# weiyithu/PV-RAFT

Hardware: NVIDIA H100
Metric: raft_sample_iters_per_sec (higher is better)
Workload: dtype f32

## Files before the change

### pvraft_b200/csrc/corr_gemm.cu

```cuda
#include "tma.cuh"
#include "wgmma.cuh"

namespace pvraft {

constexpr int kGemmThreads = 384;
constexpr int kTileM = 128, kTileN = 128, kBlockK = 32;
constexpr int kOperandBytes = kTileM * kBlockK * 4;
constexpr int kStageBytes = 4 * kOperandBytes;
constexpr int kStages = 3;
constexpr int kConsumerWarps = 8;

struct GemmParams {
    float* corr;
    int N, M, C;
    float scale;
    float rscale;
    int r0, c0;
    int tiles_m, tiles_n;
    long long ldc;
    long long n_tiles;
};

__device__ __forceinline__ float div_by_const(float x, float s, float r) {
    const float q0 = x * r;
    return fmaf(fmaf(-q0, s, x), r, q0);
}

__global__ void __launch_bounds__(kGemmThreads, 1)
k_corr_gemm(const __grid_constant__ CUtensorMap map_a_hi, const __grid_constant__ CUtensorMap map_a_lo,
            const __grid_constant__ CUtensorMap map_b_hi, const __grid_constant__ CUtensorMap map_b_lo, const GemmParams p) {
    extern __shared__ __align__(1024) unsigned char smem_raw[];
    unsigned char* tiles = SMEM_ALIGN_1024(smem_raw);
    __shared__ __align__(8) unsigned long long s_full[kStages], s_empty[kStages];
    const int warp = warp_id(), lane = lane_id();
    const int num_kb = p.C / kBlockK;
    const long long my_tiles = blockIdx.x < p.n_tiles ? (p.n_tiles - 1 - blockIdx.x) / gridDim.x + 1 : 0;

    if (warp == 0 && lane == 0) {
        prefetch_tensormap(&map_a_hi);
        prefetch_tensormap(&map_a_lo);
        prefetch_tensormap(&map_b_hi);
        prefetch_tensormap(&map_b_lo);
        for (int s = 0; s < kStages; ++s) { mbar_init(&s_full[s], 1); mbar_init(&s_empty[s], kConsumerWarps); }
        fence_mbarrier_init();
    }
    __syncthreads();
    const int tiles_per_batch = p.tiles_m * p.tiles_n;

    if (warp < 4) {
        if (warp == 0 && lane == 0) {
            int s = 0;
            unsigned phase = 0;
            for (long long i = 0; i < my_tiles; ++i) {
                const long long t = blockIdx.x + i * gridDim.x;
                const int b = (int)(t / tiles_per_batch), r = (int)(t - (long long)b * tiles_per_batch);
                const int tile_m = r / p.tiles_n, tile_n = r - tile_m * p.tiles_n;
                const int row_a = b * p.N + p.r0 + tile_m * kTileM, row_b = b * p.M + p.c0 + tile_n * kTileN;
                for (int kb = 0; kb < num_kb; ++kb) {
                    mbar_wait(&s_empty[s], phase ^ 1u);
                    unsigned char* st = tiles + (size_t)s * kStageBytes;
                    mbar_expect_tx(&s_full[s], kStageBytes);
                    tma_load_2d(st + 0 * kOperandBytes, &map_a_hi, &s_full[s], kb * kBlockK, row_a);
                    tma_load_2d(st + 1 * kOperandBytes, &map_a_lo, &s_full[s], kb * kBlockK, row_a);
                    tma_load_2d(st + 2 * kOperandBytes, &map_b_hi, &s_full[s], kb * kBlockK, row_b);
                    tma_load_2d(st + 3 * kOperandBytes, &map_b_lo, &s_full[s], kb * kBlockK, row_b);
                    if (++s == kStages) { s = 0; phase ^= 1u; }
                }
            }
        }
        return;
    }
    const int half = (warp >> 2) - 1;
    const int wq = warp & 3;
    const int a_off = half * 64 * 128;
    float acc[64];
    int s = 0, prev_s = -1;
    unsigned phase = 0;
    for (long long i = 0; i < my_tiles; ++i) {
        const long long t = blockIdx.x + i * gridDim.x;
        const int b = (int)(t / tiles_per_batch), r = (int)(t - (long long)b * tiles_per_batch);
        const int tile_m = r / p.tiles_n, tile_n = r - tile_m * p.tiles_n;
        for (int kb = 0; kb < num_kb; ++kb) {
            mbar_wait(&s_full[s], phase);
            unsigned char* st = tiles + (size_t)s * kStageBytes;
            const unsigned long long a_hi = wgmma_desc(st + 0 * kOperandBytes + a_off), a_lo = wgmma_desc(st + 1 * kOperandBytes + a_off);
            const unsigned long long b_hi = wgmma_desc(st + 2 * kOperandBytes), b_lo = wgmma_desc(st + 3 * kOperandBytes);
            wgmma_fence_regs(acc);
            wgmma_fence();
#pragma unroll
            for (int k = 0; k < kBlockK / 8; ++k) {
                wgmma_tf32<kTileN>(acc, wgmma_desc_k(a_hi, k), wgmma_desc_k(b_hi, k), (kb | k) != 0);
                wgmma_tf32<kTileN>(acc, wgmma_desc_k(a_lo, k), wgmma_desc_k(b_hi, k), 1);
                wgmma_tf32<kTileN>(acc, wgmma_desc_k(a_hi, k), wgmma_desc_k(b_lo, k), 1);
            }
            wgmma_commit();
            wgmma_wait<1>();
            if (prev_s >= 0 && lane == 0) mbar_arrive(&s_empty[prev_s]);
            prev_s = s;
            if (++s == kStages) { s = 0; phase ^= 1u; }
        }
        wgmma_wait<0>();
        wgmma_fence_regs(acc);
        if (lane == 0) mbar_arrive(&s_empty[prev_s]);
        prev_s = -1;
        const int row = tile_m * kTileM + half * 64 + wq * 16 + (lane >> 2);
        float* o = p.corr + ((size_t)b * p.tiles_m * kTileM + row) * (size_t)p.ldc + (size_t)tile_n * kTileN + 2 * (lane & 3);
        const size_t down8 = (size_t)8 * p.ldc;
#pragma unroll
        for (int j = 0; j < kTileN / 8; ++j) {
            *reinterpret_cast<float2*>(o + 8 * j) = make_float2(div_by_const(acc[4 * j + 0], p.scale, p.rscale), div_by_const(acc[4 * j + 1], p.scale, p.rscale));
            *reinterpret_cast<float2*>(o + down8 + 8 * j) = make_float2(div_by_const(acc[4 * j + 2], p.scale, p.rscale), div_by_const(acc[4 * j + 3], p.scale, p.rscale));
        }
    }
}

__global__ void k_tf32_split(const float* __restrict__ x, long long n, float* __restrict__ hi, float* __restrict__ lo) {
    const long long i = ((long long)blockIdx.x * blockDim.x + threadIdx.x) * 4;
    if (i >= n) return;
    const float4 v = *reinterpret_cast<const float4*>(x + i);
    float h[4], l[4];
    const float in[4] = {v.x, v.y, v.z, v.w};
#pragma unroll
    for (int q = 0; q < 4; ++q) {
        unsigned hb, lb;
        asm("cvt.rna.tf32.f32 %0, %1;" : "=r"(hb) : "f"(in[q]));
        h[q] = __uint_as_float(hb);
        asm("cvt.rna.tf32.f32 %0, %1;" : "=r"(lb) : "f"(in[q] - h[q]));
        l[q] = __uint_as_float(lb);
    }
    *reinterpret_cast<float4*>(hi + i) = make_float4(h[0], h[1], h[2], h[3]);
    *reinterpret_cast<float4*>(lo + i) = make_float4(l[0], l[1], l[2], l[3]);
}

static int launch_gemm(const float* a_hi, const float* a_lo, const float* b_hi, const float* b_lo, int B, int N, int M, int C, int r0,
                       int tiles_m, int c0, int tiles_n, float* corr, long long ldc, cudaStream_t st) {
    int rc;
    CUtensorMap ma_hi, ma_lo, mb_hi, mb_lo;
    const long long rows_a = (long long)B * N, rows_b = (long long)B * M;
    if ((rc = make_tensor_map(&ma_hi, a_hi, rows_a, C, C, kTileM, "corr_matmul")) ||
        (rc = make_tensor_map(&ma_lo, a_lo, rows_a, C, C, kTileM, "corr_matmul")) ||
        (rc = make_tensor_map(&mb_hi, b_hi, rows_b, C, C, kTileN, "corr_matmul")) ||
        (rc = make_tensor_map(&mb_lo, b_lo, rows_b, C, C, kTileN, "corr_matmul")))
        return rc;
    GemmParams p{};
    p.corr = corr; p.N = N; p.M = M; p.C = C;
    p.scale = sqrtf((float)C);
    p.rscale = (float)(1.0 / (double)p.scale);
    p.r0 = r0; p.c0 = c0;
    p.tiles_m = tiles_m; p.tiles_n = tiles_n;
    p.ldc = ldc;
    p.n_tiles = (long long)B * tiles_m * tiles_n;
    const size_t smem = (size_t)kStages * kStageBytes + 1024;
    if ((rc = opt_in_smem(k_corr_gemm, smem))) return rc;
    const int grid = (int)(p.n_tiles < sm_count() ? p.n_tiles : sm_count());
    k_corr_gemm<<<grid, kGemmThreads, smem, st>>>(ma_hi, ma_lo, mb_hi, mb_lo, p);
    return check_launch("corr_gemm");
}

static void launch_split(const float* x, long long n, float* hi, float* lo, cudaStream_t st) {
    k_tf32_split<<<(unsigned)((n / 4 + 255) / 256), 256, 0, st>>>(x, n, hi, lo);
}

}

using namespace pvraft;

extern "C" int64_t pvraft_corr_matmul_workspace_bytes(int B, int N, int M, int C) {
    if (B <= 0 || N <= 0 || M <= 0 || C <= 0) return 0;
    return (int64_t)2 * B * ((int64_t)N + M) * C * (int64_t)sizeof(float);
}

extern "C" int pvraft_corr_matmul_fwd(const float* fmap1, const float* fmap2, int B, int N, int M, int C, float* corr, void* workspace,
                                      void* stream) {
    if (!fmap1 || !fmap2 || !corr || !workspace) return fail(PVRAFT_ERR_BAD_ARG, "corr_matmul: null pointer");
    if (B <= 0 || N <= 0 || M <= 0 || C <= 0) return fail(PVRAFT_ERR_BAD_ARG, "corr_matmul: bad shape");
    if (N % kTileM || M % kTileN || C % kBlockK)
        return fail(PVRAFT_ERR_UNSUPPORTED, "corr_matmul: N=%d and M=%d must be multiples of 128 and C=%d of 32", N, M, C);
    if (B > 65535 || N / kTileM > 65535 || M / kTileN > 65535) return fail(PVRAFT_ERR_UNSUPPORTED, "corr_matmul: grid too large");
    cudaStream_t st = (cudaStream_t)stream;
    const long long na = (long long)B * N * C, nb = (long long)B * M * C;
    float* a_hi = reinterpret_cast<float*>(workspace);
    float* a_lo = a_hi + na;
    float* b_hi = a_lo + na;
    float* b_lo = b_hi + nb;
    launch_split(fmap1, na, a_hi, a_lo, st);
    launch_split(fmap2, nb, b_hi, b_lo, st);
    const int rc = check_launch("tf32_split");
    if (rc) return rc;
    return launch_gemm(a_hi, a_lo, b_hi, b_lo, B, N, M, C, 0, N / kTileM, 0, M / kTileN, corr, M, st);
}

extern "C" int pvraft_tf32_split_fwd(const float* x, int64_t n, float* hi, float* lo, void* stream) {
    if (!x || !hi || !lo || n <= 0) return fail(PVRAFT_ERR_BAD_ARG, "tf32_split: bad argument");
    if (n % 4 || ((uintptr_t)x | (uintptr_t)hi | (uintptr_t)lo) % 16)
        return fail(PVRAFT_ERR_UNSUPPORTED, "tf32_split: n=%lld must be a multiple of 4 and the buffers 16-byte aligned", (long long)n);
    launch_split(x, n, hi, lo, (cudaStream_t)stream);
    return check_launch("tf32_split");
}

extern "C" int pvraft_corr_matmul_window_fwd(const float* a_hi, const float* a_lo, const float* b_hi, const float* b_lo, int B, int N,
                                             int M, int C, int r0, int rows, int c0, int cols, float* corr, int64_t ldc, void* stream) {
    if (!a_hi || !a_lo || !b_hi || !b_lo || !corr) return fail(PVRAFT_ERR_BAD_ARG, "corr_matmul_window: null pointer");
    if (B <= 0 || N <= 0 || M <= 0 || C <= 0 || rows <= 0 || cols <= 0 || r0 < 0 || c0 < 0)
        return fail(PVRAFT_ERR_BAD_ARG, "corr_matmul_window: bad shape");
    if (N % kTileM || M % kTileN || C % kBlockK || r0 % kTileM || c0 % kTileN)
        return fail(PVRAFT_ERR_UNSUPPORTED, "corr_matmul_window: N=%d, M=%d, r0=%d and c0=%d must be multiples of 128 and C=%d of 32", N,
                    M, r0, c0, C);
    const int tiles_m = (rows + kTileM - 1) / kTileM, tiles_n = (cols + kTileN - 1) / kTileN;
    if (rows > N - r0 || cols > M - c0 || r0 + tiles_m * kTileM > N || c0 + tiles_n * kTileN > M)
        return fail(PVRAFT_ERR_UNSUPPORTED, "corr_matmul_window: rows [%d, %d) x columns [%d, %d), whole tiles, exceed N=%d x M=%d", r0,
                    r0 + tiles_m * kTileM, c0, c0 + tiles_n * kTileN, N, M);
    if (ldc < (int64_t)tiles_n * kTileN || ldc % 4)
        return fail(PVRAFT_ERR_UNSUPPORTED, "corr_matmul_window: ldc=%lld (need a multiple of 4, >= %d)", (long long)ldc, tiles_n * kTileN);
    if ((long long)B * N > 0x7fffffffLL || (long long)B * M > 0x7fffffffLL)
        return fail(PVRAFT_ERR_UNSUPPORTED, "corr_matmul_window: B*N=%lld / B*M=%lld operand rows", (long long)B * N, (long long)B * M);
    return launch_gemm(a_hi, a_lo, b_hi, b_lo, B, N, M, C, r0, tiles_m, c0, tiles_n, corr, ldc, (cudaStream_t)stream);
}
```

### pvraft_b200/csrc/corr_topk.cu

```cuda
#include "common.cuh"

namespace pvraft {

constexpr int kTopkThreads = 256;

__device__ __forceinline__ int padded(int i) { return i + (i >> 5); }

__global__ void __launch_bounds__(kTopkThreads) k_corr_topk(const float* __restrict__ corr, int M, long long ld, int K,
                                                            float* __restrict__ val, int32_t* __restrict__ idx, long long ld_out,
                                                            int col_base, const int32_t* __restrict__ ids) {
    extern __shared__ __align__(16) unsigned char smem_raw[];
    unsigned* s_key = reinterpret_cast<unsigned*>(smem_raw);
    __shared__ int s_hist[256];
    __shared__ unsigned s_prefix, s_need;
    __shared__ unsigned s_warp[kTopkThreads / 32];
    const size_t row = blockIdx.x;
    const float* src = corr + row * (size_t)ld;
    const int tid = threadIdx.x, lane = tid & 31, w = tid >> 5;
    for (int i = tid; i < M; i += kTopkThreads) s_key[padded(i)] = ord_key(__ldg(src + i));
    if (tid == 0) { s_prefix = 0u; s_need = (unsigned)K; }
    for (int pass = 0; pass < 4; ++pass) {
        const int shift = 24 - 8 * pass;
        s_hist[tid] = 0;
        __syncthreads();
        const unsigned prefix = s_prefix;
        const unsigned mask = pass == 0 ? 0u : (0xFFFFFFFFu << (shift + 8));
        for (int i = tid; i < M; i += kTopkThreads) {
            const unsigned k = s_key[padded(i)];
            if ((k & mask) == prefix) atomicAdd(&s_hist[(k >> shift) & 0xFF], 1);
        }
        __syncthreads();
        if (w == 0) {
            int h[8], mine = 0;
#pragma unroll
            for (int q = 0; q < 8; ++q) { h[q] = s_hist[lane * 8 + q]; mine += h[q]; }
            int above = mine;
#pragma unroll
            for (int o = 1; o < 32; o <<= 1) {
                const int a = __shfl_down_sync(kFull, above, o);
                if (lane + o < 32) above += a;
            }
            const int need = (int)s_need;
            const int higher = above - mine;
            const bool here = higher < need && above >= need;
            if (here) {
                int acc = higher, bin = 7;
                for (; bin > 0; --bin) {
                    if (acc + h[bin] >= need) break;
                    acc += h[bin];
                }
                s_need = (unsigned)(need - acc);
                s_prefix = prefix | ((unsigned)(lane * 8 + bin) << shift);
            }
        }
        __syncthreads();
    }
    const unsigned T = s_prefix;
    const int need_eq = (int)s_need;
    const int seg = (M + kTopkThreads - 1) / kTopkThreads;
    const int c0 = tid * seg, c1 = min(M, c0 + seg);
    unsigned n_gt = 0, n_eq = 0;
    for (int i = c0; i < c1; ++i) {
        const unsigned k = s_key[padded(i)];
        n_gt += k > T ? 1u : 0u;
        n_eq += k == T ? 1u : 0u;
    }
    unsigned packed = n_gt | (n_eq << 16), incl = packed;
#pragma unroll
    for (int o = 1; o < 32; o <<= 1) {
        const unsigned a = __shfl_up_sync(kFull, incl, o);
        if (lane >= o) incl += a;
    }
    if (lane == 31) s_warp[w] = incl;
    __syncthreads();
    unsigned base = 0;
    for (int q = 0; q < w; ++q) base += s_warp[q];
    const unsigned excl = base + incl - packed;
    const int gt_before = (int)(excl & 0xFFFFu), eq_before = (int)(excl >> 16);
    int pos = gt_before + min(eq_before, need_eq);
    int eq_seen = eq_before;
    for (int i = c0; i < c1; ++i) {
        const unsigned k = s_key[padded(i)];
        bool keep = k > T;
        if (k == T) { keep = eq_seen < need_eq; ++eq_seen; }
        if (keep) {
            val[row * ld_out + pos] = ord_float(k);
            idx[row * ld_out + pos] = ids ? __ldg(ids + row * ld + i) : col_base + i;
            ++pos;
        }
    }
}

__global__ void __launch_bounds__(kTopkThreads) k_corr_topk_vec(const float* __restrict__ corr, int M, long long ld, int K,
                                                                float* __restrict__ val, int32_t* __restrict__ idx, long long ld_out,
                                                                int col_base, const int32_t* __restrict__ ids) {
    extern __shared__ __align__(16) unsigned char smem_raw[];
    uint4* s_key = reinterpret_cast<uint4*>(smem_raw);
    constexpr int kCand = 1024;
    __shared__ int s_hist[2048 + kTopkThreads];
    __shared__ unsigned s_cand[kCand];
    __shared__ int s_wsum[kTopkThreads / 32];
    __shared__ unsigned s_scan[kTopkThreads / 32][7];
    __shared__ unsigned s_prefix;
    __shared__ int s_need;
    const int tid = threadIdx.x, lane = tid & 31, w = tid >> 5;
    const size_t row = blockIdx.x;
    const float4* src = reinterpret_cast<const float4*>(corr + row * (size_t)ld);
#pragma unroll
    for (int j = 0; j < 8; ++j) {
        const int c4 = j * kTopkThreads + tid;
        uint4 kk = make_uint4(0u, 0u, 0u, 0u);
        if (c4 * 4 < M) {
            const float4 v = __ldg(src + c4);
            kk = make_uint4(ord_key(v.x), ord_key(v.y), ord_key(v.z), ord_key(v.w));
        }
        s_key[c4] = kk;
    }
    const int sink = 2048 + tid;
    auto find_bin = [&](unsigned prefix, int shift, int need) {
        int h[8], mine = 0;
#pragma unroll
        for (int q = 0; q < 8; ++q) { h[q] = s_hist[tid * 8 + q]; mine += h[q]; }
        int incl = mine;
#pragma unroll
        for (int o = 1; o < 32; o <<= 1) {
            const int a = __shfl_down_sync(kFull, incl, o);
            if (lane + o < 32) incl += a;
        }
        if (lane == 0) s_wsum[w] = incl;
        __syncthreads();
        int above = incl;
        for (int ww = w + 1; ww < kTopkThreads / 32; ++ww) above += s_wsum[ww];
        const int higher = above - mine;
        if (higher < need && above >= need) {
            int acc = higher, bin = 7;
            for (; bin > 0; --bin) {
                if (acc + h[bin] >= need) break;
                acc += h[bin];
            }
            s_need = need - acc;
            s_prefix = prefix | ((unsigned)(tid * 8 + bin) << shift);
        }
        __syncthreads();
    };
    for (int i = tid; i < 2048; i += kTopkThreads) s_hist[i] = 0;
    __syncthreads();
#pragma unroll
    for (int j = 0; j < 8; ++j) {
        const uint4 kk = s_key[j * kTopkThreads + tid];
        atomicAdd(&s_hist[kk.x >> 21], 1);
        atomicAdd(&s_hist[kk.y >> 21], 1);
        atomicAdd(&s_hist[kk.z >> 21], 1);
        atomicAdd(&s_hist[kk.w >> 21], 1);
    }
    __syncthreads();
    find_bin(0u, 21, K);
    unsigned prefix = s_prefix;
    int need = s_need;
    int ncand = 0;
    {
        const unsigned top = prefix >> 21;
        int mine = 0;
#pragma unroll
        for (int j = 0; j < 8; ++j) {
            const uint4 kk = s_key[j * kTopkThreads + tid];
            mine += ((kk.x >> 21) == top) + ((kk.y >> 21) == top) + ((kk.z >> 21) == top) + ((kk.w >> 21) == top);
        }
        int incl = mine;
#pragma unroll
        for (int o = 1; o < 32; o <<= 1) {
            const int a = __shfl_up_sync(kFull, incl, o);
            if (lane >= o) incl += a;
        }
        if (lane == 31) s_wsum[w] = incl;
        __syncthreads();
        int at = incl - mine, total = 0;
        for (int ww = 0; ww < kTopkThreads / 32; ++ww) {
            const int a = s_wsum[ww];
            total += a;
            if (ww < w) at += a;
        }
        ncand = total;
        if (total <= kCand && mine > 0) {
#pragma unroll
            for (int j = 0; j < 8; ++j) {
                const uint4 kk = s_key[j * kTopkThreads + tid];
                const unsigned ke[4] = {kk.x, kk.y, kk.z, kk.w};
#pragma unroll
                for (int e = 0; e < 4; ++e) {
                    const bool hit = (ke[e] >> 21) == top;
                    if (hit) s_cand[at] = ke[e];
                    at += hit ? 1 : 0;
                }
            }
        }
    }
    __syncthreads();
#pragma unroll 1
    for (int pass = 1; pass < 3; ++pass) {
        const int shift = pass == 1 ? 10 : 0;
        const unsigned digit_mask = pass == 1 ? 0x7FFu : 0x3FFu;
        const unsigned hi_mask = 0xFFFFFFFFu << (shift + (pass == 1 ? 11 : 10));
        for (int i = tid; i < 2048; i += kTopkThreads) s_hist[i] = 0;
        __syncthreads();
        if (ncand <= kCand) {
            for (int i = tid; i < ncand; i += kTopkThreads) {
                const unsigned k = s_cand[i];
                atomicAdd(&s_hist[(k & hi_mask) == prefix ? (int)((k >> shift) & digit_mask) : sink], 1);
            }
        } else {
#pragma unroll
            for (int j = 0; j < 8; ++j) {
                const uint4 kk = s_key[j * kTopkThreads + tid];
                atomicAdd(&s_hist[(kk.x & hi_mask) == prefix ? (int)((kk.x >> shift) & digit_mask) : sink], 1);
                atomicAdd(&s_hist[(kk.y & hi_mask) == prefix ? (int)((kk.y >> shift) & digit_mask) : sink], 1);
                atomicAdd(&s_hist[(kk.z & hi_mask) == prefix ? (int)((kk.z >> shift) & digit_mask) : sink], 1);
                atomicAdd(&s_hist[(kk.w & hi_mask) == prefix ? (int)((kk.w >> shift) & digit_mask) : sink], 1);
            }
        }
        __syncthreads();
        find_bin(prefix, shift, need);
        prefix = s_prefix;
        need = s_need;
    }
    const unsigned T = prefix;
    const int need_eq = need;
    unsigned cnt[7] = {0u, 0u, 0u, 0u, 0u, 0u, 0u};
#pragma unroll
    for (int j = 0; j < 8; ++j) {
        const uint4 kk = s_key[j * kTopkThreads + tid];
        const unsigned g = (kk.x > T) + (kk.y > T) + (kk.z > T) + (kk.w > T);
        const unsigned q = (kk.x == T) + (kk.y == T) + (kk.z == T) + (kk.w == T);
        cnt[j / 3] += g << (11 * (j % 3));
        cnt[3 + j / 2] += q << (16 * (j % 2));
    }
    unsigned inc[7];
#pragma unroll
    for (int i = 0; i < 7; ++i) inc[i] = cnt[i];
#pragma unroll
    for (int o = 1; o < 32; o <<= 1) {
#pragma unroll
        for (int i = 0; i < 7; ++i) {
            const unsigned a = __shfl_up_sync(kFull, inc[i], o);
            if (lane >= o) inc[i] += a;
        }
    }
    if (lane == 31) {
#pragma unroll
        for (int i = 0; i < 7; ++i) s_scan[w][i] = inc[i];
    }
    __syncthreads();
    unsigned tot[7] = {0u, 0u, 0u, 0u, 0u, 0u, 0u}, before[7];
#pragma unroll
    for (int i = 0; i < 7; ++i) before[i] = inc[i] - cnt[i];
    for (int ww = 0; ww < kTopkThreads / 32; ++ww) {
#pragma unroll
        for (int i = 0; i < 7; ++i) {
            const unsigned a = s_scan[ww][i];
            tot[i] += a;
            if (ww < w) before[i] += a;
        }
    }
    __syncthreads();
    unsigned* s_oval = s_cand;
    int* s_oidx = s_hist;
    int base_gt = 0, base_eq = 0;
#pragma unroll
    for (int j = 0; j < 8; ++j) {
        const int sh = 11 * (j % 3), sq = 16 * (j % 2);
        int gt_before = base_gt + (int)((before[j / 3] >> sh) & 0x7FFu);
        int eq_before = base_eq + (int)((before[3 + j / 2] >> sq) & 0xFFFFu);
        base_gt += (int)((tot[j / 3] >> sh) & 0x7FFu);
        base_eq += (int)((tot[3 + j / 2] >> sq) & 0xFFFFu);
        const unsigned mine = ((cnt[j / 3] >> sh) & 0x7FFu) | ((cnt[3 + j / 2] >> sq) & 0xFFFFu);
        if (mine == 0u) continue;
        const int col = (j * kTopkThreads + tid) * 4;
        const uint4 kk = s_key[j * kTopkThreads + tid];
        const unsigned ke[4] = {kk.x, kk.y, kk.z, kk.w};
#pragma unroll
        for (int e = 0; e < 4; ++e) {
            const unsigned key = ke[e];
            const bool gt = key > T, eq = key == T;
            if (gt || (eq && eq_before < need_eq)) {
                const int pos = gt_before + min(eq_before, need_eq);
                s_oval[pos] = key;
                s_oidx[pos] = col + e;
            }
            gt_before += gt ? 1 : 0;
            eq_before += eq ? 1 : 0;
        }
    }
    __syncthreads();
    float* vrow = val + row * (size_t)ld_out;
    int32_t* irow = idx + row * (size_t)ld_out;
    const int32_t* idrow = ids ? ids + row * (size_t)ld : nullptr;
    for (int i = tid; i < K; i += kTopkThreads) {
        vrow[i] = ord_float(s_oval[i]);
        irow[i] = idrow ? __ldg(idrow + s_oidx[i]) : col_base + s_oidx[i];
    }
}

static int launch_topk(const float* corr, long long rows, int M, long long ld, int K, int col_base, const int32_t* ids, float* val,
                       int32_t* idx, long long ld_out, cudaStream_t st) {
    if (M <= 8192 && M % 4 == 0 && ld % 4 == 0 && (uintptr_t)corr % 16 == 0) {
        k_corr_topk_vec<<<(unsigned)rows, kTopkThreads, 8 * kTopkThreads * sizeof(uint4), st>>>(corr, M, ld, K, val, idx, ld_out, col_base, ids);
        return check_launch("corr_topk");
    }
    const size_t smem = (size_t)(M + (M >> 5) + 4) * 4;
    int rc;
    if ((rc = opt_in_smem(k_corr_topk, smem))) return rc;
    k_corr_topk<<<(unsigned)rows, kTopkThreads, smem, st>>>(corr, M, ld, K, val, idx, ld_out, col_base, ids);
    return check_launch("corr_topk");
}

}

using namespace pvraft;

extern "C" int pvraft_corr_topk_fwd(const float* corr, int B, int N, int M, int K, float* val, int32_t* idx, void* stream) {
    if (!corr || !val || !idx) return fail(PVRAFT_ERR_BAD_ARG, "corr_topk: null pointer");
    if (B <= 0 || N <= 0 || M <= 0) return fail(PVRAFT_ERR_BAD_ARG, "corr_topk: bad shape");
    if (K < 1 || K > M || K > 1024) return fail(PVRAFT_ERR_UNSUPPORTED, "corr_topk: K=%d with M=%d (need 1 <= K <= min(M,1024))", K, M);
    if (M > 49152) return fail(PVRAFT_ERR_UNSUPPORTED, "corr_topk: M=%d columns (max 49152)", M);
    const long long rows = (long long)B * N;
    if (rows > 0x7fffffffLL) return fail(PVRAFT_ERR_UNSUPPORTED, "corr_topk: too many rows");
    return launch_topk(corr, rows, M, M, K, 0, nullptr, val, idx, K, (cudaStream_t)stream);
}

extern "C" int pvraft_corr_topk_window_fwd(const float* corr, int rows, int cols, int64_t ld, int K, int col_base, const int32_t* cand_ids,
                                           float* val, int32_t* idx, int64_t ld_out, void* stream) {
    if (!corr || !val || !idx) return fail(PVRAFT_ERR_BAD_ARG, "corr_topk_window: null pointer");
    if (rows <= 0 || cols <= 0 || ld < cols || col_base < 0) return fail(PVRAFT_ERR_BAD_ARG, "corr_topk_window: bad shape");
    if (K < 1 || K > cols || K > 1024 || ld_out < K)
        return fail(PVRAFT_ERR_UNSUPPORTED, "corr_topk_window: K=%d with cols=%d, ld_out=%lld (need 1 <= K <= min(cols,1024), ld_out >= K)", K,
                    cols, (long long)ld_out);
    if (cols > 49152) return fail(PVRAFT_ERR_UNSUPPORTED, "corr_topk_window: cols=%d (max 49152)", cols);
    if (!cand_ids && (long long)col_base + cols > 0x7fffffffLL) return fail(PVRAFT_ERR_UNSUPPORTED, "corr_topk_window: column ids overflow");
    return launch_topk(corr, rows, cols, ld, K, col_base, cand_ids, val, idx, ld_out, (cudaStream_t)stream);
}
```

### pvraft_b200/ops.py

```python
import ctypes as C
import threading
import types
import weakref
from typing import NamedTuple

import torch

from . import _lib
from ._lib import (ACT_LRELU, ACT_NONE, ACT_RELU, IN_GN, IN_GN_MINMAX, IN_PLAIN, KNN, MOMENTS, check, lib)

launch_count = 0


def _stream():
    return C.c_void_p(torch.cuda.current_stream().cuda_stream)


def _p(t, dtype=torch.float32):
    if t is None or not isinstance(t, torch.Tensor):
        return t
    if not t.is_cuda:
        raise _lib.PvraftError('pvraft_b200 kernels need CUDA tensors (no CPU fallback exists)')
    if t.device.index != torch.cuda.current_device():
        raise _lib.PvraftError(f'tensor on {t.device} but the current CUDA device is {torch.cuda.current_device()}: the kernels '
                               'launch on the current device -- wrap the call in `with torch.cuda.device(t.device):`')
    if t.dtype != dtype and not (isinstance(dtype, tuple) and t.dtype in dtype):
        raise TypeError(f'expected {dtype}, got {t.dtype}')
    if not t.is_contiguous():
        raise ValueError('expected a contiguous tensor')
    return t.data_ptr()


_DTYPES = {'float': torch.float32, 'double': torch.float64, 'int32_t': torch.int32, 'int': torch.int32, 'uint8_t': torch.uint8,
           'int8_t': torch.int8, 'uint16_t': (torch.bfloat16, torch.int16), 'void': torch.uint8}


def _count(rc, what):
    global launch_count
    check(rc, what)
    launch_count += 1


def _convert(i, d, value, namespace):
    if d.pointee is None:
        return value
    if d.pointee in _lib.STRUCTS:
        namespace[f'_t{i}'] = _lib.STRUCTS[d.pointee]
        return f'_byref({value}) if isinstance({value}, _t{i}) else {value}'
    namespace[f'_d{i}'] = _DTYPES[d.pointee]
    return f'_p({value}, _d{i})'


def _compile(src, name, namespace):
    namespace['_byref'] = C.byref
    signature = ', '.join(f'{k}={k}' for k in namespace)
    exec(src.replace('@DEFAULTS@', signature), globals(), namespace)
    return namespace[name]


_UNCOUNTED = ('pvraft_tc_weight_split', 'pvraft_tc_weight_bf16')


def _entry(name, params):
    launches = bool(params) and params[-1].name == 'stream' and params[-1].pointee == 'void'
    params = params[:-1] if launches else params
    namespace = {}
    args = [f'a{i}' for i in range(len(params))]
    call = ', '.join(_convert(i, d, f'a{i}', namespace) for i, d in enumerate(params))
    if launches:
        body = f"{'check' if name in _UNCOUNTED else '_count'}(lib().{name}({call}{', ' if params else ''}_stream()), {name!r})"
    else:
        body = f'return lib().{name}({call})'
    return _compile(f"def {name}({', '.join(args + ['*'])}, @DEFAULTS@):\n    {body}\n", name, namespace)


def _packer(struct, fields):
    namespace = {'_S': struct}
    lines = ['if _s is None:\n        _s = _S()']
    for i, d in enumerate(fields):
        if d.length > 1:
            lines.append(f'if {d.name} is not None:\n        for _i, _v in enumerate({d.name}):\n'
                         f'            _s.{d.name}[_i] = {_convert(i, d, "_v", namespace)}')
        else:
            lines.append(f'if {d.name} is not None:\n        _s.{d.name} = {_convert(i, d, d.name, namespace)}')
    lines.append('return _s')
    names = ', '.join(f'{d.name}=None' for d in fields)
    return _compile(f'def {struct.__name__}(_s=None, /, *, {names}, @DEFAULTS@):\n    ' + '\n    '.join(lines) + '\n',
                    struct.__name__, namespace)


abi = types.SimpleNamespace(**{name[len('pvraft_'):]: _entry(name, params) for name, (_, params) in _lib.FUNCTIONS.items()})
pack = types.SimpleNamespace(**{cls.__name__: _packer(cls, _lib.STRUCT_FIELDS[s]) for s, cls in _lib.STRUCTS.items()})


def deterministic():
    return torch.are_deterministic_algorithms_enabled()


def _det_workspace(size_fn, *size_args, device):
    if not deterministic():
        return None
    return torch.zeros(int(size_fn(*size_args)), dtype=torch.uint8, device=device)


_TLS = threading.local()


class stats_arena:

    def __init__(self, b, device, blocks):
        self.buf = [torch.zeros(blocks, b, 8, 2, dtype=torch.float64, device=device), 0]

    def __enter__(self):
        self.prev = getattr(_TLS, 'arena', None)
        _TLS.arena = self.buf
        return self

    def __exit__(self, *exc):
        _TLS.arena = self.prev
        return False


class bf16_compute:

    def __init__(self, enabled=True):
        self.enabled = bool(enabled)

    def __enter__(self):
        self.prev = getattr(_TLS, 'bf16', False)
        _TLS.bf16 = self.enabled
        return self

    def __exit__(self, *exc):
        _TLS.bf16 = self.prev
        return False


def bf16_compute_active():
    return bool(getattr(_TLS, 'bf16', False))


def new_stats(b, device, n=1):
    arena = getattr(_TLS, 'arena', None)
    if arena is not None:
        buf, pos = arena
        if pos + n <= buf.shape[0] and buf.shape[1] == b and buf.device == torch.device(device):
            arena[1] = pos + n
            return buf[pos:pos + n]
    return torch.zeros(n, b, 8, 2, dtype=torch.float64, device=device)


def corr_reorder(val, idx):
    b, n, k = val.shape
    val_out, idx_out = torch.empty_like(val), torch.empty_like(idx)
    abi.corr_reorder(val, idx, b * n, k, val_out, idx_out)
    return val_out, idx_out


def corr_state_pack_bf16(val, idx, m=None):
    m = int(idx.shape[1]) if m is None else int(m)
    if m > 65536:
        raise ValueError(f'uint16 candidate ids need a second cloud of at most 65536 points (N2 <= 65536), got {m}')
    v16 = torch.empty(val.shape, dtype=torch.bfloat16, device=val.device)
    i16 = torch.empty(idx.shape, dtype=torch.int16, device=idx.device)
    abi.corr_state_pack_bf16(val, idx, val.numel(), v16, i16)
    return v16, i16


def corr_matmul(fmap1_pm, fmap2_pm):
    b, n, c = fmap1_pm.shape
    m = fmap2_pm.shape[1]
    if fmap2_pm.shape != (b, m, c):
        raise ValueError(f'corr_matmul: feature maps {tuple(fmap1_pm.shape)} and {tuple(fmap2_pm.shape)}')
    corr = torch.empty(b, n, m, dtype=torch.float32, device=fmap1_pm.device)
    ws = _workspace(abi.corr_matmul_workspace_bytes(b, n, m, c), fmap1_pm.device)
    abi.corr_matmul_fwd(fmap1_pm, fmap2_pm, b, n, m, c, corr, ws)
    return corr


def corr_topk(corr, k):
    b, n, m = corr.shape
    val = torch.empty(b, n, k, dtype=torch.float32, device=corr.device)
    idx = torch.empty(b, n, k, dtype=torch.int32, device=corr.device)
    abi.corr_topk_fwd(corr, b, n, m, k, val, idx)
    return val, idx


def corr_dense(fmap1_pm, fmap2_pm):
    n, m = fmap1_pm.shape[1], fmap2_pm.shape[1]
    pad_n, pad_m = (-n) % 128, (-m) % 128
    if pad_n == 0 and pad_m == 0:
        return corr_matmul(fmap1_pm, fmap2_pm)
    f1 = torch.nn.functional.pad(fmap1_pm, (0, 0, 0, pad_n)).contiguous()
    f2 = torch.nn.functional.pad(fmap2_pm, (0, 0, 0, pad_m)).contiguous()
    return corr_matmul(f1, f2)[:, :n, :m].contiguous()


CORR_ROW_MAX = 49152
CORR_SLAB_CAP = 1 << 30


class CorrPlan(NamedTuple):
    dense: bool
    windows: tuple
    row_blocks: tuple
    ld: int
    slab_bytes: int


def _pad128(x):
    return (x + 127) // 128 * 128


def corr_plan(b, n, m, c, k, window=CORR_ROW_MAX, cap=CORR_SLAB_CAP):
    if min(b, n, m, c, k) <= 0:
        raise ValueError(f'corr_plan: bad shape B={b} N={n} M={m} C={c} K={k}')
    if window % 128 or not 0 < window <= CORR_ROW_MAX:
        raise ValueError(f'corr_plan: window={window} must be a multiple of 128 and at most {CORR_ROW_MAX}')
    if m <= window:
        return CorrPlan(True, ((0, m),), ((0, n),), _pad128(m), 4 * b * _pad128(n) * _pad128(m))
    if k > m:
        raise ValueError(f'truncate_k={k} exceeds the number of points {m}')
    w = -(-m // window)
    if w * k > CORR_ROW_MAX:
        raise ValueError(f'a cloud of {m} points needs {w} column windows, and their {w * k} candidates per row exceed the '
                         f'{CORR_ROW_MAX} the merge step can stage (truncate_k={k}: at most {CORR_ROW_MAX // k * window} points)')
    width = _pad128(-(-m // w))
    windows = tuple((i * width, min(width, m - i * width)) for i in range(w))
    if windows[-1][1] < k:
        raise ValueError(f'corr_plan: the last column window has {windows[-1][1]} columns, fewer than truncate_k={k}')
    per_row = 4 * width + 8 * w * k
    rows = max(128, cap // per_row // 128 * 128)
    nb = -(-_pad128(n) // rows)
    rows = _pad128(-(-n // nb))
    row_blocks = tuple((r0, min(rows, n - r0)) for r0 in range(0, n, rows))
    return CorrPlan(False, windows, row_blocks, width, rows * per_row)


def corr_build(fmap1_pm, fmap2_pm, k, plan=None):
    b, n, c = fmap1_pm.shape
    m = fmap2_pm.shape[1]
    if fmap2_pm.dim() != 3 or fmap2_pm.shape[0] != b or fmap2_pm.shape[2] != c:
        raise ValueError(f'corr_build: feature maps {tuple(fmap1_pm.shape)} and {tuple(fmap2_pm.shape)} (same batch and channels)')
    if k > m:
        raise ValueError(f'truncate_k={k} exceeds the number of points {m} of the second cloud')
    if c % 32 != 0:
        raise NotImplementedError(f'calculate_corr: {c} feature channels (the wgmma GEMM needs a multiple of 32; the model has 128)')
    plan = corr_plan(b, n, m, c, k) if plan is None else plan
    if plan.dense:
        return corr_topk(corr_dense(fmap1_pm, fmap2_pm), k)
    dev = fmap1_pm.device
    npad, mpad = _pad128(n), _pad128(m)
    ws_a = torch.empty(2, b, npad, c, dtype=torch.float32, device=dev)
    ws_b = torch.empty(2, b, mpad, c, dtype=torch.float32, device=dev)
    for ws, f, rows_f in ((ws_a, fmap1_pm, n), (ws_b, fmap2_pm, m)):
        for s in range(b):
            abi.tf32_split_fwd(f[s], rows_f * c, ws[0, s], ws[1, s])
    nw = len(plan.windows)
    wk = nw * k
    rows = max(r for _, r in plan.row_blocks)
    slab = torch.empty(_pad128(rows), plan.ld, dtype=torch.float32, device=dev)
    cand_val = torch.empty(rows, wk, dtype=torch.float32, device=dev)
    cand_idx = torch.empty(rows, wk, dtype=torch.int32, device=dev)
    val = torch.empty(b, n, k, dtype=torch.float32, device=dev)
    idx = torch.empty(b, n, k, dtype=torch.int32, device=dev)
    for s in range(b):
        split = (ws_a[0, s], ws_a[1, s], ws_b[0, s], ws_b[1, s])
        for r0, nr in plan.row_blocks:
            for j, (c0, nc) in enumerate(plan.windows):
                abi.corr_matmul_window_fwd(*split, 1, npad, mpad, c, r0, nr, c0, nc, slab, plan.ld)
                abi.corr_topk_window_fwd(slab, nr, nc, plan.ld, k, c0, None, cand_val.view(-1)[j * k:], cand_idx.view(-1)[j * k:], wk)
            abi.corr_topk_window_fwd(cand_val, nr, wk, wk, k, 0, cand_idx, val[s, r0:r0 + nr], idx[s, r0:r0 + nr], k)
    return val, idx


def _table_rows(xyz2_pad, b):
    if xyz2_pad.dim() != 3 or xyz2_pad.shape[0] != b or xyz2_pad.shape[2] != 4:
        raise ValueError(f'expected a gather table [B={b},M,4], got {tuple(xyz2_pad.shape)}')
    return int(xyz2_pad.shape[1])


def check_pair(xyz1, xyz2, truncate_k):
    if xyz1.dim() != 3 or xyz1.shape[-1] != 3 or xyz2.dim() != 3 or xyz2.shape[-1] != 3:
        raise ValueError(f'expected p = [xyz1 [B,N1,3], xyz2 [B,N2,3]], got {tuple(xyz1.shape)} and {tuple(xyz2.shape)}')
    if xyz1.shape[0] != xyz2.shape[0]:
        raise ValueError(f'xyz1 {tuple(xyz1.shape)} and xyz2 {tuple(xyz2.shape)} must have the same batch size')
    n1, n2 = int(xyz1.shape[1]), int(xyz2.shape[1])
    if min(n1, n2) < KNN:
        raise ValueError(f'need at least {KNN} points per cloud, got N1={n1} and N2={n2}')
    if truncate_k > n2:
        raise ValueError(f'truncate_k={truncate_k} exceeds the number of points {n2} of the second cloud')


def xyz_pad(xyz):
    b, n, _ = xyz.shape
    out = torch.empty(b, n, 4, dtype=torch.float32, device=xyz.device)
    abi.xyz_pad_fwd(xyz, b * n, out)
    return out


def corr_lookup(corr_val, corr_idx, xyz2_pad, coords, levels, base_scale, vox=None, knn_sel=None, moments=None,
                want_slots=False, want_cube=False, vox_ld=None):
    b, n, k = corr_val.shape
    m = _table_rows(xyz2_pad, b)
    dev = corr_val.device
    if vox_ld is None:
        vox_ld = (levels * 27 + 3) // 4 * 4
    if vox is None:
        vox = torch.empty(b, n, vox_ld, dtype=torch.float32, device=dev)
    if knn_sel is None:
        knn_sel = torch.empty(b, n, KNN, 4, dtype=torch.float32, device=dev)
    if moments is None:
        moments = new_stats(b, dev, 1).view(b, MOMENTS) if MOMENTS == 16 else torch.zeros(b, MOMENTS, dtype=torch.float64, device=dev)
    slots = torch.empty(b, n, KNN, dtype=torch.int32, device=dev) if want_slots else None
    cube = torch.empty(b, n, k, levels, dtype=torch.int8, device=dev) if want_cube else None
    fn = abi.corr_lookup_bf16_fwd if corr_val.dtype == torch.bfloat16 else abi.corr_lookup_fwd
    ws = _det_workspace(abi.corr_lookup_det_workspace_bytes, b, device=dev)
    fn(corr_val, corr_idx, xyz2_pad, coords, b, n, m, k, levels, float(base_scale), vox, vox.shape[-1], knn_sel, slots, moments, cube, ws)
    return dict(vox=vox, knn_sel=knn_sel, moments=moments, knn_slot=slots, cube=cube)


def linear(x, weight, bias=None, *, cin=None, w_ld=0, w_cin=0, in_mode=IN_PLAIN, in_min=None, in_stats=None, in_gamma=None,
           in_beta=None, in_count=0.0, in_act=ACT_NONE, in_slope=0.0, out_act=ACT_NONE, out=None, out_stats=None,
           residual=None, cout=None):
    b, n, c = x.shape
    cin = c if cin is None else cin
    cout = weight.shape[0] if cout is None else cout
    if out is None:
        out = torch.empty(b, n, cout, dtype=torch.float32, device=x.device)
    a = pack.LinearArgs(in_=x, in_min=in_min, in_stats=in_stats, in_gamma=in_gamma, in_beta=in_beta, in_count=float(in_count),
                        in_mode=in_mode, in_act=in_act, in_slope=float(in_slope), weight=weight, w_ld=int(w_ld), w_cin=int(w_cin),
                        bias=bias, residual=residual, out_act=out_act, out=out, out_stats=out_stats, B=b, N=n, cin=cin, cout=cout)
    ws = _det_workspace(abi.linear_det_workspace_bytes, b, device=x.device) if out_stats is not None else None
    abi.linear_fwd(a, ws)
    return out


_TC_WEIGHTS = {}
TC_PLAIN, TC_GRU_ZR, TC_GRU_Q, TC_FLOW = 0, 1, 2, 3


def tc_weights(weights, col0=0, cols=None, k_pad=None, kcat=False, transposed=None, bf16=None):
    if torch.is_tensor(weights):
        weights = (weights,)
    bf16 = bf16_compute_active() if bf16 is None else bool(bf16)
    key = tuple(id(w) for w in weights) + (col0, cols, k_pad, kcat, transposed, bf16)
    hit = _TC_WEIGHTS.get(key)
    if hit is not None:
        refs, versions, ptrs, result = hit
        if all(r() is w and w._version == v and w.data_ptr() == p for r, w, v, p in zip(refs, weights, versions, ptrs)):
            return result
    _TLS.unsettled = 3
    mats = [w.detach().reshape(w.shape[0], -1) for w in weights]
    if transposed is not None:
        mats = [m.t()[transposed[0]:transposed[1]].contiguous() for m in mats]
    if kcat:
        mats = [torch.cat(mats, 1).contiguous()]
    ld = mats[0].shape[1]
    ncols = ld - col0 if cols is None else cols
    kp = (ncols + 31) // 32 * 32 if k_pad is None else k_pad
    rows = sum(m.shape[0] for m in mats)
    n_pad = (rows + 15) // 16 * 16
    alloc = torch.empty if n_pad == rows else torch.zeros
    if bf16:
        hi, lo = alloc(n_pad, kp, dtype=torch.bfloat16, device=mats[0].device), None
    else:
        hi = alloc(n_pad, kp, dtype=torch.float32, device=mats[0].device)
        lo = alloc(n_pad, kp, dtype=torch.float32, device=mats[0].device)
    r0 = 0
    for m in mats:
        if bf16:
            abi.tc_weight_bf16(m.contiguous(), m.shape[0], ncols, ld, col0, m.shape[0], kp, hi[r0:])
        else:
            abi.tc_weight_split(m.contiguous(), m.shape[0], ncols, ld, col0, m.shape[0], kp, hi[r0:], lo[r0:])
        r0 += m.shape[0]
    if len(_TC_WEIGHTS) > 512:
        _TC_WEIGHTS.clear()
    result = (hi, lo, n_pad, rows)
    _TC_WEIGHTS[key] = (tuple(weakref.ref(w) for w in weights), tuple(w._version for w in weights),
                        tuple(w.data_ptr() for w in weights), result)
    return result


_DERIVED = {}


def derived(tensors, tag, fn):
    key = tuple(id(t) for t in tensors) + (tag,)
    hit = _DERIVED.get(key)
    if hit is not None:
        refs, versions, ptrs, value = hit
        if all(r() is t and t._version == v and t.data_ptr() == p for r, t, v, p in zip(refs, tensors, versions, ptrs)):
            return value
    _TLS.unsettled = 3
    value = fn(*tensors)
    if len(_DERIVED) > 512:
        _DERIVED.clear()
    _DERIVED[key] = (tuple(weakref.ref(t) for t in tensors), tuple(t._version for t in tensors),
                     tuple(t.data_ptr() for t in tensors), value)
    return value


KNN_SORT_MAX_N = 16384


def point_order(points):
    b, n, _ = points.shape
    ws_bytes = int(abi.knn_workspace_bytes(b, n))
    if ws_bytes <= 0 or n < 64 or n > KNN_SORT_MAX_N:
        return morton_order(points).to(torch.int32).contiguous()
    ws = _workspace(ws_bytes, points.device)
    perm = torch.empty(b, n, dtype=torch.int32, device=points.device)
    abi.point_order_fwd(points, b, n, perm, ws)
    return perm


def morton_order(points):
    lo, hi = points.amin(1, keepdim=True), points.amax(1, keepdim=True)
    q = ((points - lo) / (hi - lo).clamp_min(1e-12) * 1023.0).long().clamp_(0, 1023)

    def spread(v):
        v = (v | (v << 16)) & 0x030000FF
        v = (v | (v << 8)) & 0x0300F00F
        v = (v | (v << 4)) & 0x030C30C3
        return (v | (v << 2)) & 0x09249249

    code = spread(q[..., 0]) | (spread(q[..., 1]) << 1) | (spread(q[..., 2]) << 2)
    return torch.sort(code, dim=1, stable=True).indices


def tc_supported(n_points, *channels):
    return n_points % 128 == 0 and all(c % 32 == 0 for c in channels)


def tc_linear(sources, w, bias=None, *, in_min=None, in_stats=None, in_gamma=None, in_beta=None, in_count=0.0,
              in_act=ACT_NONE, in_slope=0.0, out_act=ACT_NONE, residual=None, out=None, out_stats=None, epilogue=TC_PLAIN,
              bias2=None, out2=None, h=None, z=None, cout=None, tail=None, w3=None, b3=None, coords1=None, coords2=None,
              coords2_out=None, flow_out=None):
    hi, lo, n_pad, rows = w
    b, n, _ = sources[0].shape
    cout = rows if cout is None else cout
    if out is None:
        out = torch.empty(b, n, cout + (3 if tail is not None else 0), dtype=torch.float32, device=sources[0].device)
    a = pack.TcLinearArgs(in_=sources, in_channels=[src.shape[-1] for src in sources], in_min=in_min, in_stats=in_stats,
                          in_gamma=in_gamma, in_beta=in_beta, in_count=float(in_count), in_act=in_act, in_slope=float(in_slope),
                          w_hi=None if lo is None else hi, w_lo=lo, w_bf16=hi if lo is None else None, n_pad=n_pad, cout=cout,
                          bias=bias, bias2=bias2, out_act=out_act, residual=residual, out=out, out2=out2, h=h, z=z,
                          out_stats=out_stats, epilogue=epilogue, B=b, N=n, tail=tail, w3=w3, b3=b3, coords1=coords1,
                          coords2=coords2, coords2_out=coords2_out, flow_out=flow_out)
    pending = getattr(_TLS, 'unsettled', 0)
    a.params_settled = 1 if pending == 0 else 0
    if pending:
        _TLS.unsettled = pending - 1
    ws = _det_workspace(abi.tc_linear_det_workspace_bytes, b, device=out.device) if out_stats is not None else None
    abi.tc_linear_fwd(a, ws)
    return out


fuse_update_chain = True


def update_chain(y1, gn, kfeat, cflow, flow, net, inp, weights, biases):
    b, n, _ = net.shape
    net_out, p_out = torch.empty_like(net), torch.empty_like(net)
    b_cc, b_m, b_z, b_r, b_q = biases
    abi.update_chain_fwd(pack.UpdateChainArgs(y1=y1, y1_stats=gn['in_stats'], gn_gamma=gn['in_gamma'], gn_beta=gn['in_beta'],
                                              gn_count=float(gn['in_count']), gn_slope=float(gn['in_slope']), kfeat=kfeat,
                                              cflow=cflow, flow=flow, net=net, inp=inp,
                                              w_hi=[None if lo is None else hi for hi, lo, _, _ in weights],
                                              w_lo=[lo for _, lo, _, _ in weights],
                                              w_bf16=[hi if lo is None else None for hi, lo, _, _ in weights], b_cc=b_cc, b_m=b_m,
                                              b_z=b_z, b_r=b_r, b_q=b_q, net_out=net_out, p_out=p_out, B=b, N=n,
                                              hidden=net.shape[-1], context=inp.shape[-1], y1_channels=y1.shape[-1]))
    return net_out, p_out


def gn_act(x, stats, gamma, beta, count, act=ACT_LRELU, slope=0.1, transpose_out=False, slope_dev=None):
    b, n, c = x.shape
    out = torch.empty((b, c, n) if transpose_out else (b, n, c), dtype=torch.float32, device=x.device)
    abi.gn_act_fwd(x, stats, gamma, beta, float(count), act, float(slope), b, n, c, int(transpose_out), out, slope_dev)
    return out


def transpose(x):
    b, r, c = x.shape
    out = torch.empty(b, c, r, dtype=torch.float32, device=x.device)
    abi.transpose_fwd(x, b, r, c, out)
    return out


def corr_feature(args):
    abi.corr_feature_fwd(args)


def knn_branch(args):
    abi.knn_branch_fwd(args)


def gru(args):
    abi.gru_fwd(args)


def flow_out(args):
    abi.flow_out_fwd(args)


def edge_plan(nbr, order=None):
    b, n, _ = nbr.shape
    rec = int(abi.edge_plan_bytes(1, 1))
    tiles = int(abi.edge_plan_bytes(1, n)) // rec
    plan = torch.empty(b, tiles, rec, dtype=torch.uint8, device=nbr.device)
    abi.edge_plan_fwd(nbr, order, b, n, plan)
    return plan


def setconv_edge(fc1p, nbr, edge_feats, w_fc1, cin, stats, ymax=None, ymin=None, order=None, plan=None):
    b, n, c = fc1p.shape
    if ymax is None:
        ymax = torch.empty_like(fc1p)
    if ymin is None:
        ymin = torch.empty_like(fc1p)
    if plan is None:
        plan = edge_plan(nbr, order)
    elif plan.shape[0] != b or plan.numel() != int(abi.edge_plan_bytes(b, n)):
        raise ValueError(f'edge plan of shape {tuple(plan.shape)} does not belong to a graph of {b} x {n} points')
    ws = _det_workspace(abi.setconv_edge_det_workspace_bytes, b, device=fc1p.device)
    abi.setconv_edge_fwd(fc1p, nbr, edge_feats, w_fc1, cin, b, n, c, ymax, ymin, stats, order, plan, ws)
    return ymax, ymin


def knn(xyz, query, k, mode=0, want_rel=False, use_sweep=True):
    b, n, _ = xyz.shape
    s = query.shape[1]
    out = torch.empty(b, s, k, dtype=torch.int32, device=xyz.device)
    rel = torch.empty(b, s, k, 3, dtype=torch.float32, device=xyz.device) if want_rel else None
    ws_bytes = int(abi.knn_workspace_bytes(b, n)) if use_sweep else 0
    ws = _workspace(ws_bytes, xyz.device) if ws_bytes > 0 else None
    abi.knn_fwd(xyz, query, b, n, s, k, mode, out, rel, ws)
    return (out, rel) if want_rel else out


def linear_wgrad(x, dy, dw, db=None):
    rows = x.shape[0] * x.shape[1]
    ws = _det_workspace(abi.linear_wgrad_det_workspace_bytes, x.shape[-1], dy.shape[-1], device=x.device)
    abi.linear_wgrad(x, dy, rows, x.shape[-1], dy.shape[-1], dw, dw.shape[-1], db, ws)


def tc_wgrad_bf16(x, dy, dw, db=None):
    rows = x.shape[0] * x.shape[1]
    ws = _det_workspace(abi.tc_wgrad_bf16_det_workspace_bytes, x.shape[-1], dy.shape[-1], device=x.device)
    abi.tc_wgrad_bf16(x, dy, rows, x.shape[-1], dy.shape[-1], dw, dw.shape[-1], db, ws)


def linear_bwd_small(x, dy, w, dw, db=None, want_dx=False):
    rows = x.shape[0] * x.shape[1]
    dx = torch.empty_like(x) if want_dx else None
    ws = _det_workspace(abi.linear_bwd_small_det_workspace_bytes, x.shape[-1], dy.shape[-1], device=x.device)
    abi.linear_bwd_small(x, dy, w, rows, x.shape[-1], dy.shape[-1], w.shape[-1], dw, dw.shape[-1], db, dx, ws)
    return dx


def gn_act_maxk(x, stats, gamma, beta, count, act, slope, slope_dev=None):
    b, rows, c = x.shape
    y = torch.empty(b, rows // 32, c, dtype=torch.float32, device=x.device)
    arg = torch.empty(b, rows // 32, c, dtype=torch.uint8, device=x.device)
    abi.gn_act_maxk_fwd(x, stats, gamma, beta, float(count), act, float(slope), b, rows // 32, c, y, arg, slope_dev)
    return y, arg


def gn_act_bwd(x, dy, stats, gamma, beta, count, act, slope, want_dslope=False, slope_dev=None, arg=None):
    b, rows, c = x.shape
# ... 426 lines not shown
```

Baseline: 9969.

## Use PDL launches and L2-sized row blocks for dense correlation path

Launches the correlation GEMM and top-k kernels with programmatic dependent launch, so each kernel's prologue can overlap the previous kernel's tail. The dense plan now streams row blocks sized to about 32 MB through a slab that should stay in L2, with a single-window fast path that writes top-k directly, instead of materializing the full correlation matrix. It also replaces the per-batch TF32 split launches with one launch per feature map. The risks are more launches from the row-block loop and a change in how the split workspace is laid out.

```diff
diff --git a/pvraft_b200/csrc/corr_gemm.cu b/pvraft_b200/csrc/corr_gemm.cu
--- a/pvraft_b200/csrc/corr_gemm.cu
+++ b/pvraft_b200/csrc/corr_gemm.cu
@@ -35,6 +35,7 @@
     const int warp = warp_id(), lane = lane_id();
     const int num_kb = p.C / kBlockK;
     const long long my_tiles = blockIdx.x < p.n_tiles ? (p.n_tiles - 1 - blockIdx.x) / gridDim.x + 1 : 0;
+    pdl_trigger();
 
     if (warp == 0 && lane == 0) {
         prefetch_tensormap(&map_a_hi);
@@ -45,6 +46,7 @@
         fence_mbarrier_init();
     }
     __syncthreads();
+    pdl_wait();
     const int tiles_per_batch = p.tiles_m * p.tiles_n;
 
     if (warp < 4) {
@@ -153,7 +155,7 @@
     const size_t smem = (size_t)kStages * kStageBytes + 1024;
     if ((rc = opt_in_smem(k_corr_gemm, smem))) return rc;
     const int grid = (int)(p.n_tiles < sm_count() ? p.n_tiles : sm_count());
-    k_corr_gemm<<<grid, kGemmThreads, smem, st>>>(ma_hi, ma_lo, mb_hi, mb_lo, p);
+    launch_pdl(k_corr_gemm, grid, kGemmThreads, smem, st, ma_hi, ma_lo, mb_hi, mb_lo, p);
     return check_launch("corr_gemm");
 }
 
diff --git a/pvraft_b200/csrc/corr_topk.cu b/pvraft_b200/csrc/corr_topk.cu
--- a/pvraft_b200/csrc/corr_topk.cu
+++ b/pvraft_b200/csrc/corr_topk.cu
@@ -14,6 +14,8 @@
     __shared__ int s_hist[256];
     __shared__ unsigned s_prefix, s_need;
     __shared__ unsigned s_warp[kTopkThreads / 32];
+    pdl_trigger();
+    pdl_wait();
     const size_t row = blockIdx.x;
     const float* src = corr + row * (size_t)ld;
     const int tid = threadIdx.x, lane = tid & 31, w = tid >> 5;
@@ -104,6 +106,8 @@
     __shared__ unsigned s_prefix;
     __shared__ int s_need;
     const int tid = threadIdx.x, lane = tid & 31, w = tid >> 5;
+    pdl_trigger();
+    pdl_wait();
     const size_t row = blockIdx.x;
     const float4* src = reinterpret_cast<const float4*>(corr + row * (size_t)ld);
 #pragma unroll
@@ -303,13 +307,14 @@
 static int launch_topk(const float* corr, long long rows, int M, long long ld, int K, int col_base, const int32_t* ids, float* val,
                        int32_t* idx, long long ld_out, cudaStream_t st) {
     if (M <= 8192 && M % 4 == 0 && ld % 4 == 0 && (uintptr_t)corr % 16 == 0) {
-        k_corr_topk_vec<<<(unsigned)rows, kTopkThreads, 8 * kTopkThreads * sizeof(uint4), st>>>(corr, M, ld, K, val, idx, ld_out, col_base, ids);
+        launch_pdl(k_corr_topk_vec, (int)rows, kTopkThreads, 8 * kTopkThreads * sizeof(uint4), st, corr, M, ld, K, val, idx, ld_out, col_base,
+                   ids);
         return check_launch("corr_topk");
     }
     const size_t smem = (size_t)(M + (M >> 5) + 4) * 4;
     int rc;
     if ((rc = opt_in_smem(k_corr_topk, smem))) return rc;
-    k_corr_topk<<<(unsigned)rows, kTopkThreads, smem, st>>>(corr, M, ld, K, val, idx, ld_out, col_base, ids);
+    launch_pdl(k_corr_topk, (int)rows, kTopkThreads, smem, st, corr, M, ld, K, val, idx, ld_out, col_base, ids);
     return check_launch("corr_topk");
 }
 
diff --git a/pvraft_b200/ops.py b/pvraft_b200/ops.py
--- a/pvraft_b200/ops.py
+++ b/pvraft_b200/ops.py
@@ -198,6 +198,7 @@
 
 CORR_ROW_MAX = 49152
 CORR_SLAB_CAP = 1 << 30
+CORR_L2_SLAB = 32 << 20
 
 
 class CorrPlan(NamedTuple):
@@ -210,6 +211,16 @@
 
 def _pad128(x):
     return (x + 127) // 128 * 128
+
+
+def _block_rows(n, per_row, cap):
+    rows = max(128, cap // per_row // 128 * 128)
+    nb = -(-_pad128(n) // rows)
+    return _pad128(-(-n // nb))
+
+
+def _row_blocks(n, rows):
+    return tuple((r0, min(rows, n - r0)) for r0 in range(0, n, rows))
 
 
 def corr_plan(b, n, m, c, k, window=CORR_ROW_MAX, cap=CORR_SLAB_CAP):
@@ -230,11 +241,8 @@
     if windows[-1][1] < k:
         raise ValueError(f'corr_plan: the last column window has {windows[-1][1]} columns, fewer than truncate_k={k}')
     per_row = 4 * width + 8 * w * k
-    rows = max(128, cap // per_row // 128 * 128)
-    nb = -(-_pad128(n) // rows)
-    rows = _pad128(-(-n // nb))
-    row_blocks = tuple((r0, min(rows, n - r0)) for r0 in range(0, n, rows))
-    return CorrPlan(False, windows, row_blocks, width, rows * per_row)
+    rows = _block_rows(n, per_row, cap)
+    return CorrPlan(False, windows, _row_blocks(n, rows), width, rows * per_row)
 
 
 def corr_build(fmap1_pm, fmap2_pm, k, plan=None):
@@ -247,26 +255,29 @@
     if c % 32 != 0:
         raise NotImplementedError(f'calculate_corr: {c} feature channels (the wgmma GEMM needs a multiple of 32; the model has 128)')
     plan = corr_plan(b, n, m, c, k) if plan is None else plan
-    if plan.dense:
-        return corr_topk(corr_dense(fmap1_pm, fmap2_pm), k)
+    row_blocks = _row_blocks(n, _block_rows(n, 4 * plan.ld, CORR_L2_SLAB)) if plan.dense else plan.row_blocks
     dev = fmap1_pm.device
     npad, mpad = _pad128(n), _pad128(m)
-    ws_a = torch.empty(2, b, npad, c, dtype=torch.float32, device=dev)
-    ws_b = torch.empty(2, b, mpad, c, dtype=torch.float32, device=dev)
-    for ws, f, rows_f in ((ws_a, fmap1_pm, n), (ws_b, fmap2_pm, m)):
-        for s in range(b):
-            abi.tf32_split_fwd(f[s], rows_f * c, ws[0, s], ws[1, s])
+    ws_a = torch.empty(2, b * n + npad - n, c, dtype=torch.float32, device=dev)
+    ws_b = torch.empty(2, b * m + mpad - m, c, dtype=torch.float32, device=dev)
+    abi.tf32_split_fwd(fmap1_pm, b * n * c, ws_a[0], ws_a[1])
+    abi.tf32_split_fwd(fmap2_pm, b * m * c, ws_b[0], ws_b[1])
     nw = len(plan.windows)
     wk = nw * k
-    rows = max(r for _, r in plan.row_blocks)
+    rows = max(r for _, r in row_blocks)
     slab = torch.empty(_pad128(rows), plan.ld, dtype=torch.float32, device=dev)
-    cand_val = torch.empty(rows, wk, dtype=torch.float32, device=dev)
-    cand_idx = torch.empty(rows, wk, dtype=torch.int32, device=dev)
+    if nw > 1:
+        cand_val = torch.empty(rows, wk, dtype=torch.float32, device=dev)
+        cand_idx = torch.empty(rows, wk, dtype=torch.int32, device=dev)
     val = torch.empty(b, n, k, dtype=torch.float32, device=dev)
     idx = torch.empty(b, n, k, dtype=torch.int32, device=dev)
     for s in range(b):
-        split = (ws_a[0, s], ws_a[1, s], ws_b[0, s], ws_b[1, s])
-        for r0, nr in plan.row_blocks:
+        split = (ws_a[0, s * n:], ws_a[1, s * n:], ws_b[0, s * m:], ws_b[1, s * m:])
+        for r0, nr in row_blocks:
+            if nw == 1:
+                abi.corr_matmul_window_fwd(*split, 1, npad, mpad, c, r0, nr, 0, m, slab, plan.ld)
+                abi.corr_topk_window_fwd(slab, nr, m, plan.ld, k, 0, None, val[s, r0:r0 + nr], idx[s, r0:r0 + nr], k)
+                continue
             for j, (c0, nc) in enumerate(plan.windows):
                 abi.corr_matmul_window_fwd(*split, 1, npad, mpad, c, r0, nr, c0, nc, slab, plan.ld)
                 abi.corr_topk_window_fwd(slab, nr, nc, plan.ld, k, c0, None, cand_val.view(-1)[j * k:], cand_idx.view(-1)[j * k:], wk)
```

Measured after the change: 9703 (median of 6 runs). -2.7%, worse.
